# vita-epfl/trajnetplusplusbaselines

Hardware: NVIDIA H100
Metric: pedestrian-steps/sec (higher is better)
Workload: dtype f32

## Files before the change

trajnetplusplusbaselines_b200/csrc/gates_tc.cu:

```cuda
#include <cuda.h>
#include <cuda_bf16.h>
#include <math_constants.h>
#include <cstdio>
#include <cstdlib>
#include <vector>

#include "common.cuh"
#include "wgmma.cuh"

namespace tb2 {

constexpr int kGtBM = 128;
constexpr int kGtBN = 256;
constexpr int kGtBK = 64;
constexpr int kGtStages = 2;
constexpr int kGtThreads = 384;
constexpr int kGtConsumerWarps = 8;
constexpr uint32_t kGtABytes = kGtBM * kGtBK * 2;
constexpr uint32_t kGtBBytes = kGtBN * kGtBK * 2;
constexpr uint32_t kGtStageBytes = 2 * kGtABytes + 2 * kGtBBytes;

__device__ __forceinline__ float g_sigmoid(float x) { return __fdividef(1.f, 1.f + __expf(-x)); }
__device__ __forceinline__ float g_tanh(float x) { return 1.f - __fdividef(2.f, __expf(2.f * x) + 1.f); }

struct GateTcParams {
    const float2* obs1;
    const float2* obs2;
    const float* h_in;
    const float* c_in;
    float* h_out;
    float* c_out;
    __nv_bfloat16* hs_out_hi;
    __nv_bfloat16* hs_out_lo;
    float* normal_out;
    float2* pos_out;
    const float* bg;
    const float* Wn;
    const float* bn;
    int M, P;
    int G;
};

template <int R, bool kGoal>
__global__ void __launch_bounds__(kGtThreads, 1)
lstm_gates_tc_kernel(const __grid_constant__ CUtensorMap map_emb_hi, const __grid_constant__ CUtensorMap map_emb_lo,
                     const __grid_constant__ CUtensorMap map_pool_hi, const __grid_constant__ CUtensorMap map_pool_lo,
                     const __grid_constant__ CUtensorMap map_h_hi, const __grid_constant__ CUtensorMap map_h_lo,
                     const __grid_constant__ CUtensorMap map_w_hi, const __grid_constant__ CUtensorMap map_w_lo,
                     GateTcParams p) {
    extern __shared__ __align__(1024) unsigned char smem_gt[];
    __shared__ __align__(8) uint64_t full_bar[kGtStages];
    __shared__ __align__(8) uint64_t empty_bar[kGtStages];
    __shared__ float wn_s[5][64];
    __shared__ float bg_s[4][64];
    constexpr int H = 64 * R;
    __shared__ float peer_part[R > 1 ? R - 1 : 1][kGtBM][5];

    const int wg = threadIdx.x >> 7, warp = threadIdx.x >> 5, lane = threadIdx.x & 31;
    const int rank = blockIdx.x;
    const int m0 = blockIdx.y * kGtBM;
    const int kb_pool = p.P / kGtBK;
    const int kb_emb = kGoal ? (64 + p.G) / kGtBK : 1;
    const int num_kb = kb_emb + kb_pool + H / kGtBK;
    const uint32_t ring = (smem_u32(smem_gt) + 1023u) & ~1023u;

    for (int i = threadIdx.x; i < 5 * 64; i += kGtThreads) wn_s[i / 64][i % 64] = p.Wn[(i / 64) * H + rank * 64 + (i % 64)];
    for (int i = threadIdx.x; i < 4 * 64; i += kGtThreads) bg_s[i / 64][i % 64] = p.bg[(i / 64) * H + rank * 64 + (i % 64)];

    if (threadIdx.x == 0) {
        for (int s = 0; s < kGtStages; ++s) {
            mbar_init(smem_u32(&full_bar[s]), 1);
            mbar_init(smem_u32(&empty_bar[s]), kGtConsumerWarps);
        }
        asm volatile("fence.mbarrier_init.release.cluster;" ::: "memory");
    }
    __syncthreads();
    grid_dep_wait();
    grid_dep_launch();
    asm volatile("barrier.cluster.arrive.release.aligned;" ::: "memory");
    bool waited_phase1 = false;

    const int rl = wg * 64 + (warp & 3) * 16 + (lane >> 2);
    float part[2][5] = {{0.f, 0.f, 0.f, 0.f, 0.f}, {0.f, 0.f, 0.f, 0.f, 0.f}};

    if (wg == 2) {
        if (threadIdx.x == 256) {
            for (int kb = 0; kb < num_kb; ++kb) {
                const int s = kb % kGtStages;
                const uint32_t phase = (kb / kGtStages) & 1;
                mbar_wait(smem_u32(&empty_bar[s]), phase ^ 1);
                const uint32_t bar = smem_u32(&full_bar[s]);
                const uint32_t base = ring + s * kGtStageBytes;
                mbar_expect_tx(bar, kGtStageBytes);
                const CUtensorMap *ahi, *alo;
                int ka;
                if constexpr (kGoal) {
                    if (kb < kb_emb) { ahi = &map_emb_hi; alo = &map_emb_lo; ka = kb * kGtBK; }
                    else if (kb < kb_emb + kb_pool) { ahi = &map_pool_hi; alo = &map_pool_lo; ka = (kb - kb_emb) * kGtBK; }
                    else { ahi = &map_h_hi; alo = &map_h_lo; ka = (kb - kb_emb - kb_pool) * kGtBK; }
                } else {
                    if (kb == 0) { ahi = &map_emb_hi; alo = &map_emb_lo; ka = 0; }
                    else if (kb <= kb_pool) { ahi = &map_pool_hi; alo = &map_pool_lo; ka = (kb - 1) * kGtBK; }
                    else { ahi = &map_h_hi; alo = &map_h_lo; ka = (kb - 1 - kb_pool) * kGtBK; }
                }
                tma_load_2d(base, ahi, bar, ka, m0);
                tma_load_2d(base + kGtABytes, alo, bar, ka, m0);
                tma_load_2d(base + 2 * kGtABytes, &map_w_hi, bar, kb * kGtBK, rank * kGtBN);
                tma_load_2d(base + 2 * kGtABytes + kGtBBytes, &map_w_lo, bar, kb * kGtBK, rank * kGtBN);
            }
        }
        __syncwarp();
    } else {
        float acc[kGtBN / 2];
#pragma unroll
        for (int i = 0; i < kGtBN / 2; ++i) acc[i] = 0.f;
        const uint32_t a_off = (uint32_t)wg * 64 * 128;
        for (int kb = 0; kb < num_kb; ++kb) {
            const int s = kb % kGtStages;
            const uint32_t phase = (kb / kGtStages) & 1;
            mbar_wait(smem_u32(&full_bar[s]), phase);
            const uint32_t base = ring + s * kGtStageBytes;
            const uint64_t a_hi = wgmma_desc(base + a_off);
            const uint64_t a_lo = wgmma_desc(base + kGtABytes + a_off);
            const uint64_t b_hi = wgmma_desc(base + 2 * kGtABytes);
            const uint64_t b_lo = wgmma_desc(base + 2 * kGtABytes + kGtBBytes);
            wgmma_fence();
#pragma unroll
            for (int k = 0; k < kGtBK / 16; ++k) {
                const uint64_t adv = (uint64_t)((k * 16 * 2) >> 4);
                wgmma_bf16(acc, a_hi + adv, b_hi + adv, (kb | k) != 0);
                wgmma_bf16(acc, a_hi + adv, b_lo + adv, 1u);
                wgmma_bf16(acc, a_lo + adv, b_hi + adv, 1u);
            }
            wgmma_commit();
            wgmma_wait_all();
            if (lane == 0) mbar_arrive(smem_u32(&empty_bar[s]));
        }
#pragma unroll
        for (int hr = 0; hr < 2; ++hr) {
            const int row = m0 + rl + 8 * hr;
            if (row >= p.M) continue;
            const float2 o1 = p.obs1[row], o2 = p.obs2[row];
            const bool masked = isnan(o1.x) || isnan(o2.x);
#pragma unroll
            for (int n8 = 0; n8 < 8; ++n8) {
                const int u = 8 * n8 + 2 * (lane & 3);
                const size_t o = (size_t)row * H + rank * 64 + u;
                float2 c = *reinterpret_cast<const float2*>(p.c_in + o);
                float2 h;
                if (!masked) {
                    float cn[2], hn[2];
                    const float cc[2] = {c.x, c.y};
#pragma unroll
                    for (int j = 0; j < 2; ++j) {
                        const int r = 4 * n8 + 2 * hr + j;
                        const float ig = g_sigmoid(acc[r] + bg_s[0][u + j]);
                        const float fg = g_sigmoid(acc[r + 32] + bg_s[1][u + j]);
                        const float gt = g_tanh(acc[r + 64] + bg_s[2][u + j]);
                        const float og = g_sigmoid(acc[r + 96] + bg_s[3][u + j]);
                        cn[j] = fg * cc[j] + ig * gt;
                        hn[j] = og * g_tanh(cn[j]);
#pragma unroll
                        for (int q = 0; q < 5; ++q) part[hr][q] = fmaf(hn[j], wn_s[q][u + j], part[hr][q]);
                    }
                    c = make_float2(cn[0], cn[1]);
                    h = make_float2(hn[0], hn[1]);
                } else {
                    h = *reinterpret_cast<const float2*>(p.h_in + o);
                }
                *reinterpret_cast<float2*>(p.h_out + o) = h;
                *reinterpret_cast<float2*>(p.c_out + o) = c;
                const __nv_bfloat16 h0 = __float2bfloat16_rn(h.x), h1 = __float2bfloat16_rn(h.y);
                const __nv_bfloat16 l0 = __float2bfloat16_rn(h.x - __bfloat162float(h0));
                const __nv_bfloat16 l1 = __float2bfloat16_rn(h.y - __bfloat162float(h1));
                *reinterpret_cast<uint32_t*>(p.hs_out_hi + o) =
                    (uint32_t)__bfloat16_as_ushort(h0) | ((uint32_t)__bfloat16_as_ushort(h1) << 16);
                *reinterpret_cast<uint32_t*>(p.hs_out_lo + o) =
                    (uint32_t)__bfloat16_as_ushort(l0) | ((uint32_t)__bfloat16_as_ushort(l1) << 16);
            }
        }
#pragma unroll
        for (int hr = 0; hr < 2; ++hr)
#pragma unroll
            for (int q = 0; q < 5; ++q) {
                part[hr][q] += __shfl_xor_sync(0xffffffffu, part[hr][q], 1);
                part[hr][q] += __shfl_xor_sync(0xffffffffu, part[hr][q], 2);
            }
        if (rank > 0) {
            asm volatile("barrier.cluster.wait.acquire.aligned;" ::: "memory");
            waited_phase1 = true;
            if ((lane & 3) == 0) {
#pragma unroll
                for (int hr = 0; hr < 2; ++hr) {
                    const uint32_t local = smem_u32(&peer_part[rank - 1][rl + 8 * hr][0]);
                    uint32_t remote;
                    asm volatile("mapa.shared::cluster.u32 %0, %1, %2;" : "=r"(remote) : "r"(local), "r"(0));
#pragma unroll
                    for (int q = 0; q < 5; ++q)
                        asm volatile("st.shared::cluster.f32 [%0], %1;" ::"r"(remote + 4 * q), "f"(part[hr][q]) : "memory");
                }
            }
            __syncwarp();
        }
    }
    if (!waited_phase1) asm volatile("barrier.cluster.wait.acquire.aligned;" ::: "memory");
    asm volatile("barrier.cluster.arrive.release.aligned;" ::: "memory");
    asm volatile("barrier.cluster.wait.acquire.aligned;" ::: "memory");
    if (wg < 2 && rank == 0 && (lane & 3) == 0) {
#pragma unroll
        for (int hr = 0; hr < 2; ++hr) {
            const int row = m0 + rl + 8 * hr;
            if (row >= p.M) continue;
            float* no = p.normal_out + (size_t)row * 5;
            const float2 o1 = p.obs1[row], o2 = p.obs2[row];
            if (isnan(o1.x) || isnan(o2.x)) {
#pragma unroll
                for (int q = 0; q < 5; ++q) no[q] = CUDART_NAN_F;
                if (p.pos_out) p.pos_out[row] = make_float2(CUDART_NAN_F, CUDART_NAN_F);
            } else {
                float s[5];
#pragma unroll
                for (int q = 0; q < 5; ++q) {
                    s[q] = part[hr][q];
#pragma unroll
                    for (int r = 1; r < R; ++r) s[q] += peer_part[r - 1][rl + 8 * hr][q];
                    s[q] += p.bn[q];
                }
                const float n0 = s[0], n1 = s[1];
                no[0] = n0;
                no[1] = n1;
                no[2] = 0.01f + 0.2f * g_sigmoid(s[2]);
                no[3] = 0.01f + 0.2f * g_sigmoid(s[3]);
                no[4] = 0.7f * g_sigmoid(s[4]);
                if (p.pos_out) p.pos_out[row] = make_float2(o2.x + n0, o2.y + n1);
            }
        }
    }
}

struct GoalEmbed {
    const float2* goals;
    const float* Wg;
    const float* bg;
    int G;
};

template <bool kGoal>
__global__ void embed_split_kernel(const float2* __restrict__ obs1, const float2* __restrict__ obs2,
                                   const float* __restrict__ We, const float* __restrict__ be,
                                   __nv_bfloat16* __restrict__ hi, __nv_bfloat16* __restrict__ lo, int M, int E,
                                   GoalEmbed ge) {
    grid_dep_wait();
    grid_dep_launch();
    const int idx = blockIdx.x * blockDim.x + threadIdx.x;
    const int W = kGoal ? E + ge.G : E;
    if (idx >= M * W) return;
    const int m = idx / W, k = idx - m * W;
    const float2 a = obs1[m], b = obs2[m];
    float v = 0.f;
    if (k < E - 2 && !(isnan(a.x) || isnan(b.x))) {
        const float vx = (b.x - a.x) * 4.0f, vy = (b.y - a.y) * 4.0f;
        v = fmaxf(fmaf(We[2 * k + 1], vy, fmaf(We[2 * k], vx, be[k])), 0.f);
    } else if (kGoal && k >= E && k < W - 2 && !(isnan(a.x) || isnan(b.x))) {
        const int kg = k - E;
        const float2 g = ge.goals[m];
        const float dx = b.x - g.x, dy = b.y - g.y;
        const float n = sqrtf(dx * dx + dy * dy);
        const float gx = n != 0.f ? dx / n : 0.f, gy = n != 0.f ? dy / n : 0.f;
        v = fmaxf(fmaf(ge.Wg[2 * kg + 1], gy * 4.0f, fmaf(ge.Wg[2 * kg], gx * 4.0f, ge.bg[kg])), 0.f);
    }
    const __nv_bfloat16 h = __float2bfloat16_rn(v);
    hi[idx] = h;
    lo[idx] = __float2bfloat16_rn(v - __bfloat162float(h));
}

__global__ void repack_gates_tc_kernel(const float* __restrict__ w_ih, const float* __restrict__ w_hh,
                                       __nv_bfloat16* __restrict__ hi, __nv_bfloat16* __restrict__ lo,
                                       int in_dim, int H) {
    const int K = in_dim + H;
    size_t total = (size_t)4 * H * K;
    for (size_t idx = (size_t)blockIdx.x * blockDim.x + threadIdx.x; idx < total;
         idx += (size_t)gridDim.x * blockDim.x) {
        const int k = (int)(idx % K);
        const int n = (int)(idx / K);
        const int rank = n / 256, gate = (n % 256) / 64, ul = n % 64;
        const int src = gate * H + rank * 64 + ul;
        const float v = k < in_dim ? w_ih[(size_t)src * in_dim + k] : w_hh[(size_t)src * H + (k - in_dim)];
        const __nv_bfloat16 h = __float2bfloat16_rn(v);
        hi[idx] = h;
        lo[idx] = __float2bfloat16_rn(v - __bfloat162float(h));
    }
}

int make_bf16_tile_map(CUtensorMap* map, const void* base, int rows, int cols, int box_rows);

bool gates_tc_supported(const tb2_lstm* m) {
    if (m->H % 64 != 0 || m->E != 64 || (m->E + m->G) % kGtBK != 0) return false;
    if (m->cfg.pool_type != TB2_POOL_NONE && !m->cfg.pool_to_input) return false;
    if (m->P % kGtBK != 0) return false;
    return true;
}

int launch_repack_gates_tc(const float* w_ih, const float* w_hh, void* hi, void* lo, int in_dim, int H,
                           cudaStream_t st) {
    repack_gates_tc_kernel<<<512, 256, 0, st>>>(w_ih, w_hh, (__nv_bfloat16*)hi, (__nv_bfloat16*)lo, in_dim, H);
    TB2_LAUNCH_CHECK();
    return TB2_OK;
}

int launch_embed_split(const tb2_lstm* m, int M, const float* obs1, const float* obs2, const float* goals, void* hi,
                       void* lo, cudaStream_t st) {
    const int total = M * (m->E + m->G);
    const GoalEmbed ge{(const float2*)goals, m->Wgl, m->bgl, m->G};
    {
        KernelTimer kt("embed_split", st);
        launch_pdl(m->G > 0 ? embed_split_kernel<true> : embed_split_kernel<false>, dim3((total + 255) / 256), dim3(256), 0,
                   st, (const float2*)obs1, (const float2*)obs2, (const float*)m->We, (const float*)m->be,
                   (__nv_bfloat16*)hi, (__nv_bfloat16*)lo, M, m->E, ge);
    }
    TB2_LAUNCH_CHECK();
    return TB2_OK;
}

template <int R, bool kGoal>
static int launch_gates_tc_k(const CUtensorMap& me_hi, const CUtensorMap& me_lo, const CUtensorMap& mp_hi,
                             const CUtensorMap& mp_lo, const CUtensorMap& mh_hi, const CUtensorMap& mh_lo,
                             const CUtensorMap& mw_hi, const CUtensorMap& mw_lo, const GateTcParams& p, cudaStream_t st) {
    const size_t smem = (size_t)kGtStages * kGtStageBytes + 1024;
    static DynSmemConfig configured;
    TB2_CHECK_CUDA(configured.ensure(lstm_gates_tc_kernel<R, kGoal>, smem));
    dim3 grid(R, (p.M + kGtBM - 1) / kGtBM);
    {
        KernelTimer kt("lstm_gates_tc", st);
        launch_pdl_cluster(lstm_gates_tc_kernel<R, kGoal>, grid, dim3(kGtThreads), smem, st, (unsigned)R, me_hi, me_lo,
                           mp_hi, mp_lo, mh_hi, mh_lo, mw_hi, mw_lo, p);
    }
    TB2_LAUNCH_CHECK();
    return TB2_OK;
}

template <int R>
static int launch_gates_tc_t(const CUtensorMap& me_hi, const CUtensorMap& me_lo, const CUtensorMap& mp_hi,
                             const CUtensorMap& mp_lo, const CUtensorMap& mh_hi, const CUtensorMap& mh_lo,
                             const CUtensorMap& mw_hi, const CUtensorMap& mw_lo, const GateTcParams& p, cudaStream_t st) {
    return p.G > 0 ? launch_gates_tc_k<R, true>(me_hi, me_lo, mp_hi, mp_lo, mh_hi, mh_lo, mw_hi, mw_lo, p, st)
                   : launch_gates_tc_k<R, false>(me_hi, me_lo, mp_hi, mp_lo, mh_hi, mh_lo, mw_hi, mw_lo, p, st);
}

int launch_gates_tc(const tb2_lstm* m, const tb2_layout* l, int phase, const float* obs1, const float* obs2,
                    const void* emb_hi, const void* emb_lo, const void* pool_hi, const void* pool_lo,
                    const void* hs_in_hi, const void* hs_in_lo, void* hs_out_hi, void* hs_out_lo,
                    const float* h_in, const float* c_in, float* h_out, float* c_out, float* normal_out,
                    float* pos_out, cudaStream_t st) {
    const int M = l->M;
    CUtensorMap me_hi, me_lo, mp_hi, mp_lo, mh_hi, mh_lo, mw_hi, mw_lo;
    int rc;
    if ((rc = make_bf16_tile_map(&me_hi, emb_hi, M, 64 + m->G, kGtBM))) return rc;
    if ((rc = make_bf16_tile_map(&me_lo, emb_lo, M, 64 + m->G, kGtBM))) return rc;
    if (m->P > 0) {
        if ((rc = make_bf16_tile_map(&mp_hi, pool_hi, M, m->P, kGtBM))) return rc;
        if ((rc = make_bf16_tile_map(&mp_lo, pool_lo, M, m->P, kGtBM))) return rc;
    } else {
        mp_hi = me_hi;
        mp_lo = me_lo;
    }
    if ((rc = make_bf16_tile_map(&mh_hi, hs_in_hi, M, m->H, kGtBM))) return rc;
    if ((rc = make_bf16_tile_map(&mh_lo, hs_in_lo, M, m->H, kGtBM))) return rc;
    if ((rc = make_bf16_tile_map(&mw_hi, m->Wg_hi[phase], 4 * m->H, m->K_gate, kGtBN))) return rc;
    if ((rc = make_bf16_tile_map(&mw_lo, m->Wg_lo[phase], 4 * m->H, m->K_gate, kGtBN))) return rc;
    GateTcParams p;
    p.obs1 = (const float2*)obs1;
    p.obs2 = (const float2*)obs2;
    p.h_in = h_in; p.c_in = c_in; p.h_out = h_out; p.c_out = c_out;
    p.hs_out_hi = (__nv_bfloat16*)hs_out_hi; p.hs_out_lo = (__nv_bfloat16*)hs_out_lo;
    p.normal_out = normal_out;
    p.pos_out = (float2*)pos_out;
    p.bg = m->bg[phase];
    p.Wn = m->Wn;
    p.bn = m->bn;
    p.M = M;
    p.P = m->P;
    p.G = m->G;
    switch (m->H) {
        case 64: return launch_gates_tc_t<1>(me_hi, me_lo, mp_hi, mp_lo, mh_hi, mh_lo, mw_hi, mw_lo, p, st);
        case 128: return launch_gates_tc_t<2>(me_hi, me_lo, mp_hi, mp_lo, mh_hi, mh_lo, mw_hi, mw_lo, p, st);
        case 192: return launch_gates_tc_t<3>(me_hi, me_lo, mp_hi, mp_lo, mh_hi, mh_lo, mw_hi, mw_lo, p, st);
        case 256: return launch_gates_tc_t<4>(me_hi, me_lo, mp_hi, mp_lo, mh_hi, mh_lo, mw_hi, mw_lo, p, st);
        default: break;
    }
    set_error(kHiddenDimMessage);
    return TB2_ERR_UNSUPPORTED;
}

}
```

trajnetplusplusbaselines_b200/csrc/gemm_tc.cu:

```cuda
#include <cuda.h>
#include <cuda_bf16.h>
#include <algorithm>

#include "common.cuh"
#include "wgmma.cuh"

namespace tb2 {

constexpr int kTcBM = 128;
constexpr int kTcBK = 64;
constexpr int kTcThreads = 384;
constexpr int kTcConsumerWarps = 8;
constexpr uint32_t kTcABytes = kTcBM * kTcBK * 2;
template <int BN> struct TcCfg {
    static constexpr uint32_t kBBytes = BN * kTcBK * 2;
    static constexpr uint32_t kStageBytes = 2 * kTcABytes + 2 * kBBytes;
    static constexpr int kStages = BN == 128 ? 3 : 4;
};

struct TcParams {
    const float* bias;
    float* Y;
    __nv_bfloat16* Y_hi;
    __nv_bfloat16* Y_lo;
    int M, N, K, relu;
};

__device__ __forceinline__ uint32_t pack_bf16x2(unsigned short a, unsigned short b) { return (uint32_t)a | ((uint32_t)b << 16); }

template <int kTcBN>
__global__ void __launch_bounds__(kTcThreads, 1)
dense_layer_tc_kernel(const __grid_constant__ CUtensorMap map_a_hi, const __grid_constant__ CUtensorMap map_a_lo,
                      const __grid_constant__ CUtensorMap map_b_hi, const __grid_constant__ CUtensorMap map_b_lo,
                      TcParams p) {
    constexpr int kTcStages = TcCfg<kTcBN>::kStages;
    constexpr uint32_t kTcBBytes = TcCfg<kTcBN>::kBBytes;
    constexpr uint32_t kTcStageBytes = TcCfg<kTcBN>::kStageBytes;
    extern __shared__ __align__(1024) unsigned char smem_tc[];
    __shared__ __align__(8) uint64_t full_bar[kTcStages];
    __shared__ __align__(8) uint64_t empty_bar[kTcStages];

    const int wg = threadIdx.x >> 7, warp = threadIdx.x >> 5, lane = threadIdx.x & 31;
    const int m0 = blockIdx.y * kTcBM, n0 = blockIdx.x * kTcBN;
    const int num_kb = p.K / kTcBK;
    const uint32_t ring = (smem_u32(smem_tc) + 1023u) & ~1023u;

    if (threadIdx.x == 0) {
        asm volatile("prefetch.tensormap [%0];" ::"l"(&map_a_hi) : "memory");
        asm volatile("prefetch.tensormap [%0];" ::"l"(&map_a_lo) : "memory");
        asm volatile("prefetch.tensormap [%0];" ::"l"(&map_b_hi) : "memory");
        asm volatile("prefetch.tensormap [%0];" ::"l"(&map_b_lo) : "memory");
        for (int s = 0; s < kTcStages; ++s) {
            mbar_init(smem_u32(&full_bar[s]), 1);
            mbar_init(smem_u32(&empty_bar[s]), kTcConsumerWarps);
        }
        asm volatile("fence.mbarrier_init.release.cluster;" ::: "memory");
    }
    __syncthreads();
    grid_dep_wait();
    grid_dep_launch();

    if (wg == 2) {
        if (threadIdx.x == 256) {
            for (int kb = 0; kb < num_kb; ++kb) {
                const int s = kb % kTcStages;
                const uint32_t phase = (kb / kTcStages) & 1;
                mbar_wait(smem_u32(&empty_bar[s]), phase ^ 1);
                const uint32_t bar = smem_u32(&full_bar[s]);
                const uint32_t base = ring + s * kTcStageBytes;
                mbar_expect_tx(bar, kTcStageBytes);
                tma_load_2d(base, &map_a_hi, bar, kb * kTcBK, m0);
                tma_load_2d(base + kTcABytes, &map_a_lo, bar, kb * kTcBK, m0);
                tma_load_2d(base + 2 * kTcABytes, &map_b_hi, bar, kb * kTcBK, n0);
                tma_load_2d(base + 2 * kTcABytes + kTcBBytes, &map_b_lo, bar, kb * kTcBK, n0);
            }
        }
        return;
    }
    float acc[kTcBN / 2];
#pragma unroll
    for (int i = 0; i < kTcBN / 2; ++i) acc[i] = 0.f;
    const uint32_t a_off = (uint32_t)wg * 64 * 128;
    for (int kb = 0; kb < num_kb; ++kb) {
        const int s = kb % kTcStages;
        const uint32_t phase = (kb / kTcStages) & 1;
        mbar_wait(smem_u32(&full_bar[s]), phase);
        const uint32_t base = ring + s * kTcStageBytes;
        const uint64_t a_hi = wgmma_desc(base + a_off);
        const uint64_t a_lo = wgmma_desc(base + kTcABytes + a_off);
        const uint64_t b_hi = wgmma_desc(base + 2 * kTcABytes);
        const uint64_t b_lo = wgmma_desc(base + 2 * kTcABytes + kTcBBytes);
        wgmma_fence();
#pragma unroll
        for (int k = 0; k < kTcBK / 16; ++k) {
            const uint64_t adv = (uint64_t)((k * 16 * 2) >> 4);
            wgmma_bf16(acc, a_hi + adv, b_hi + adv, (kb | k) != 0);
            wgmma_bf16(acc, a_hi + adv, b_lo + adv, 1u);
            wgmma_bf16(acc, a_lo + adv, b_hi + adv, 1u);
        }
        wgmma_commit();
        wgmma_wait_all();
        if (lane == 0) mbar_arrive(smem_u32(&empty_bar[s]));
    }
    const int row0 = m0 + wg * 64 + (warp & 3) * 16 + (lane >> 2);
    const int col0 = n0 + 2 * (lane & 3);
#pragma unroll
    for (int i = 0; i < kTcBN / 2; i += 2) {
        const int gr = row0 + 8 * ((i >> 1) & 1);
        const int gc = col0 + 8 * (i >> 2);
        float v0 = acc[i] + p.bias[gc], v1 = acc[i + 1] + p.bias[gc + 1];
        if (p.relu) { v0 = fmaxf(v0, 0.f); v1 = fmaxf(v1, 0.f); }
        if (gr >= p.M) continue;
        const size_t yoff = (size_t)gr * p.N + gc;
        if (p.Y) *reinterpret_cast<float2*>(p.Y + yoff) = make_float2(v0, v1);
        if (p.Y_hi) {
            const __nv_bfloat16 h0 = __float2bfloat16_rn(v0), h1 = __float2bfloat16_rn(v1);
            *reinterpret_cast<uint32_t*>(p.Y_hi + yoff) = pack_bf16x2(__bfloat16_as_ushort(h0), __bfloat16_as_ushort(h1));
            *reinterpret_cast<uint32_t*>(p.Y_lo + yoff) =
                pack_bf16x2(__bfloat16_as_ushort(__float2bfloat16_rn(v0 - __bfloat162float(h0))),
                            __bfloat16_as_ushort(__float2bfloat16_rn(v1 - __bfloat162float(h1))));
        }
    }
}

typedef CUresult (*EncodeTiledFn)(CUtensorMap*, CUtensorMapDataType, cuuint32_t, void*, const cuuint64_t*,
                                  const cuuint64_t*, const cuuint32_t*, const cuuint32_t*, CUtensorMapInterleave,
                                  CUtensorMapSwizzle, CUtensorMapL2promotion, CUtensorMapFloatOOBfill);

static EncodeTiledFn encode_fn() {
    static EncodeTiledFn fn = nullptr;
    if (!fn) {
        void* p = nullptr;
        cudaDriverEntryPointQueryResult q;
        if (cudaGetDriverEntryPoint("cuTensorMapEncodeTiled", &p, cudaEnableDefault, &q) == cudaSuccess &&
            q == cudaDriverEntryPointSuccess)
            fn = (EncodeTiledFn)p;
    }
    return fn;
}

int make_bf16_tile_map(CUtensorMap* map, const void* base, int rows, int cols, int box_rows) {
    struct Entry { const void* base; int rows, cols, box_rows; bool valid; CUtensorMap map; };
    static thread_local Entry cache[256] = {};
    const uintptr_t key = reinterpret_cast<uintptr_t>(base);
    Entry& e = cache[((key >> 8) ^ (key >> 17) ^ (uintptr_t)(rows * 131 + cols * 7 + box_rows)) & 255];
    if (e.valid && e.base == base && e.rows == rows && e.cols == cols && e.box_rows == box_rows) {
        *map = e.map;
        return TB2_OK;
    }
    EncodeTiledFn fn = encode_fn();
    if (!fn) { set_error("cuTensorMapEncodeTiled unavailable"); return TB2_ERR_CUDA; }
    cuuint64_t dims[2] = {(cuuint64_t)cols, (cuuint64_t)rows};
    cuuint64_t strides[1] = {(cuuint64_t)cols * 2};
    cuuint32_t box[2] = {(cuuint32_t)kTcBK, (cuuint32_t)box_rows};
    cuuint32_t estr[2] = {1, 1};
    CUresult r = fn(map, CU_TENSOR_MAP_DATA_TYPE_BFLOAT16, 2, const_cast<void*>(base), dims, strides, box, estr,
                    CU_TENSOR_MAP_INTERLEAVE_NONE, CU_TENSOR_MAP_SWIZZLE_128B, CU_TENSOR_MAP_L2_PROMOTION_L2_256B,
                    CU_TENSOR_MAP_FLOAT_OOB_FILL_NONE);
    if (r != CUDA_SUCCESS) { set_error("cuTensorMapEncodeTiled failed (" + std::to_string((int)r) + ")"); return TB2_ERR_CUDA; }
    e.base = base; e.rows = rows; e.cols = cols; e.box_rows = box_rows; e.map = *map; e.valid = true;
    return TB2_OK;
}

bool dense_tc_supported(int K, int N) { return K >= kTcBK && K % kTcBK == 0 && N % 64 == 0; }

template <int BN>
static int launch_dense_tc_t(const CUtensorMap& ma_hi, const CUtensorMap& ma_lo, const CUtensorMap& mb_hi,
                             const CUtensorMap& mb_lo, const TcParams& p, cudaStream_t st) {
    const size_t smem = (size_t)TcCfg<BN>::kStages * TcCfg<BN>::kStageBytes + 1024;
    static DynSmemConfig configured;
    TB2_CHECK_CUDA(configured.ensure(dense_layer_tc_kernel<BN>, smem));
    dim3 grid(p.N / BN, (p.M + kTcBM - 1) / kTcBM);
    {
        KernelTimer kt("dense_layer_tc", st);
        launch_pdl(dense_layer_tc_kernel<BN>, grid, dim3(kTcThreads), smem, st, ma_hi, ma_lo, mb_hi, mb_lo, p);
    }
    TB2_LAUNCH_CHECK();
    return TB2_OK;
}

int launch_dense_tc(const void* a_hi, const void* a_lo, const void* w_hi, const void* w_lo, const float* bias,
                    float* Y, void* Y_hi, void* Y_lo, int M, int K, int N, int relu, cudaStream_t st) {
    TB2_REQUIRE(dense_tc_supported(K, N), "tensor-core dense layer needs K % 64 == 0 and N % 64 == 0");
    CUtensorMap ma_hi, ma_lo, mb_hi, mb_lo;
    int rc;
    if ((rc = make_bf16_tile_map(&ma_hi, a_hi, M, K, kTcBM))) return rc;
    if ((rc = make_bf16_tile_map(&ma_lo, a_lo, M, K, kTcBM))) return rc;
    const int bn = (N % 128 == 0) ? 128 : 64;
    if ((rc = make_bf16_tile_map(&mb_hi, w_hi, N, K, bn))) return rc;
    if ((rc = make_bf16_tile_map(&mb_lo, w_lo, N, K, bn))) return rc;
    TcParams p;
    p.bias = bias;
    p.Y = Y;
    p.Y_hi = (__nv_bfloat16*)Y_hi;
    p.Y_lo = (__nv_bfloat16*)Y_lo;
    p.M = M;
    p.N = N;
    p.K = K;
    p.relu = relu;
    return bn == 128 ? launch_dense_tc_t<128>(ma_hi, ma_lo, mb_hi, mb_lo, p, st)
                     : launch_dense_tc_t<64>(ma_hi, ma_lo, mb_hi, mb_lo, p, st);
}

__global__ void split_bf16_kernel(const float* __restrict__ src, __nv_bfloat16* __restrict__ hi,
                                  __nv_bfloat16* __restrict__ lo, size_t n) {
    for (size_t i = (size_t)blockIdx.x * blockDim.x + threadIdx.x; i < n; i += (size_t)gridDim.x * blockDim.x) {
        const float v = src[i];
        const __nv_bfloat16 h = __float2bfloat16_rn(v);
        hi[i] = h;
        lo[i] = __float2bfloat16_rn(v - __bfloat162float(h));
    }
}

int launch_split_bf16(const float* src, void* hi, void* lo, size_t n, cudaStream_t st) {
    if (n == 0) return TB2_OK;
    const unsigned blocks = (unsigned)std::min<size_t>((n + 255) / 256, 1184);
    split_bf16_kernel<<<blocks, 256, 0, st>>>(src, (__nv_bfloat16*)hi, (__nv_bfloat16*)lo, n);
    TB2_LAUNCH_CHECK();
    return TB2_OK;
}

}
```

trajnetplusplusbaselines_b200/csrc/wgmma.cuh:

```cuda
#pragma once
#include <cuda.h>
#include <stdint.h>

namespace tb2 {

__device__ __forceinline__ uint32_t smem_u32(const void* p) { return (uint32_t)__cvta_generic_to_shared(p); }

__device__ __forceinline__ void mbar_init(uint32_t bar, uint32_t count) {
    asm volatile("mbarrier.init.shared::cta.b64 [%0], %1;" ::"r"(bar), "r"(count));
}
__device__ __forceinline__ void mbar_expect_tx(uint32_t bar, uint32_t bytes) {
    asm volatile("mbarrier.arrive.expect_tx.shared::cta.b64 _, [%0], %1;" ::"r"(bar), "r"(bytes) : "memory");
}
__device__ __forceinline__ void mbar_arrive(uint32_t bar) {
    asm volatile("mbarrier.arrive.shared::cta.b64 _, [%0];" ::"r"(bar) : "memory");
}
__device__ __forceinline__ void mbar_wait(uint32_t bar, uint32_t parity) {
    asm volatile(
        "{\n"
        ".reg .pred p;\n"
        "WAIT_LOOP:\n"
        "mbarrier.try_wait.parity.shared::cta.b64 p, [%0], %1;\n"
        "@p bra WAIT_DONE;\n"
        "bra WAIT_LOOP;\n"
        "WAIT_DONE:\n"
        "}\n" ::"r"(bar), "r"(parity) : "memory");
}
__device__ __forceinline__ void tma_load_2d(uint32_t dst, const CUtensorMap* map, uint32_t bar, int c0, int c1) {
    asm volatile(
        "cp.async.bulk.tensor.2d.shared::cluster.global.mbarrier::complete_tx::bytes [%0], [%1, {%3, %4}], [%2];"
        ::"r"(dst), "l"(map), "r"(bar), "r"(c0), "r"(c1) : "memory");
}

__device__ __forceinline__ uint64_t wgmma_desc(uint32_t smem_addr) {
    uint64_t d = 0;
    d |= (uint64_t)((smem_addr & 0x3FFFF) >> 4);
    d |= (uint64_t)1 << 16;
    d |= (uint64_t)(1024 >> 4) << 32;
    d |= (uint64_t)1 << 62;
    return d;
}
__device__ __forceinline__ void wgmma_fence() { asm volatile("wgmma.fence.sync.aligned;" ::: "memory"); }
__device__ __forceinline__ void wgmma_commit() { asm volatile("wgmma.commit_group.sync.aligned;" ::: "memory"); }
__device__ __forceinline__ void wgmma_wait_all() { asm volatile("wgmma.wait_group.sync.aligned 0;" ::: "memory"); }

__device__ __forceinline__ void wgmma_bf16(float (&d)[32], uint64_t a, uint64_t b, uint32_t accumulate) {
    asm volatile(
        "{\n"
        ".reg .pred p;\n"
        "setp.ne.b32 p, %34, 0;\n"
        "wgmma.mma_async.sync.aligned.m64n64k16.f32.bf16.bf16 "
        "{%0, %1, %2, %3, %4, %5, %6, %7, %8, %9, %10, %11, %12, %13, %14, %15, %16, %17, %18, %19, %20, %21, %22, %23, %24, %25, %26, %27, %28, %29, %30, %31}, "
        "%32, %33, p, 1, 1, 0, 0;\n"
        "}\n"
        : "+f"(d[0]), "+f"(d[1]), "+f"(d[2]), "+f"(d[3]), "+f"(d[4]), "+f"(d[5]), "+f"(d[6]), "+f"(d[7]),
          "+f"(d[8]), "+f"(d[9]), "+f"(d[10]), "+f"(d[11]), "+f"(d[12]), "+f"(d[13]), "+f"(d[14]), "+f"(d[15]),
          "+f"(d[16]), "+f"(d[17]), "+f"(d[18]), "+f"(d[19]), "+f"(d[20]), "+f"(d[21]), "+f"(d[22]), "+f"(d[23]),
          "+f"(d[24]), "+f"(d[25]), "+f"(d[26]), "+f"(d[27]), "+f"(d[28]), "+f"(d[29]), "+f"(d[30]), "+f"(d[31])
        : "l"(a), "l"(b), "r"(accumulate));
}
__device__ __forceinline__ void wgmma_bf16(float (&d)[64], uint64_t a, uint64_t b, uint32_t accumulate) {
    asm volatile(
        "{\n"
        ".reg .pred p;\n"
        "setp.ne.b32 p, %66, 0;\n"
        "wgmma.mma_async.sync.aligned.m64n128k16.f32.bf16.bf16 "
        "{%0, %1, %2, %3, %4, %5, %6, %7, %8, %9, %10, %11, %12, %13, %14, %15, %16, %17, %18, %19, %20, %21, %22, %23, %24, %25, %26, %27, %28, %29, %30, %31, %32, %33, %34, %35, %36, %37, %38, %39, %40, %41, %42, %43, %44, %45, %46, %47, %48, %49, %50, %51, %52, %53, %54, %55, %56, %57, %58, %59, %60, %61, %62, %63}, "
        "%64, %65, p, 1, 1, 0, 0;\n"
        "}\n"
        : "+f"(d[0]), "+f"(d[1]), "+f"(d[2]), "+f"(d[3]), "+f"(d[4]), "+f"(d[5]), "+f"(d[6]), "+f"(d[7]),
          "+f"(d[8]), "+f"(d[9]), "+f"(d[10]), "+f"(d[11]), "+f"(d[12]), "+f"(d[13]), "+f"(d[14]), "+f"(d[15]),
          "+f"(d[16]), "+f"(d[17]), "+f"(d[18]), "+f"(d[19]), "+f"(d[20]), "+f"(d[21]), "+f"(d[22]), "+f"(d[23]),
          "+f"(d[24]), "+f"(d[25]), "+f"(d[26]), "+f"(d[27]), "+f"(d[28]), "+f"(d[29]), "+f"(d[30]), "+f"(d[31]),
          "+f"(d[32]), "+f"(d[33]), "+f"(d[34]), "+f"(d[35]), "+f"(d[36]), "+f"(d[37]), "+f"(d[38]), "+f"(d[39]),
          "+f"(d[40]), "+f"(d[41]), "+f"(d[42]), "+f"(d[43]), "+f"(d[44]), "+f"(d[45]), "+f"(d[46]), "+f"(d[47]),
          "+f"(d[48]), "+f"(d[49]), "+f"(d[50]), "+f"(d[51]), "+f"(d[52]), "+f"(d[53]), "+f"(d[54]), "+f"(d[55]),
          "+f"(d[56]), "+f"(d[57]), "+f"(d[58]), "+f"(d[59]), "+f"(d[60]), "+f"(d[61]), "+f"(d[62]), "+f"(d[63])
        : "l"(a), "l"(b), "r"(accumulate));
}
__device__ __forceinline__ void wgmma_bf16(float (&d)[128], uint64_t a, uint64_t b, uint32_t accumulate) {
    asm volatile(
        "{\n"
        ".reg .pred p;\n"
        "setp.ne.b32 p, %130, 0;\n"
        "wgmma.mma_async.sync.aligned.m64n256k16.f32.bf16.bf16 "
        "{%0, %1, %2, %3, %4, %5, %6, %7, %8, %9, %10, %11, %12, %13, %14, %15, %16, %17, %18, %19, %20, %21, %22, %23, %24, %25, %26, %27, %28, %29, %30, %31, %32, %33, %34, %35, %36, %37, %38, %39, %40, %41, %42, %43, %44, %45, %46, %47, %48, %49, %50, %51, %52, %53, %54, %55, %56, %57, %58, %59, %60, %61, %62, %63, %64, %65, %66, %67, %68, %69, %70, %71, %72, %73, %74, %75, %76, %77, %78, %79, %80, %81, %82, %83, %84, %85, %86, %87, %88, %89, %90, %91, %92, %93, %94, %95, %96, %97, %98, %99, %100, %101, %102, %103, %104, %105, %106, %107, %108, %109, %110, %111, %112, %113, %114, %115, %116, %117, %118, %119, %120, %121, %122, %123, %124, %125, %126, %127}, "
        "%128, %129, p, 1, 1, 0, 0;\n"
        "}\n"
        : "+f"(d[0]), "+f"(d[1]), "+f"(d[2]), "+f"(d[3]), "+f"(d[4]), "+f"(d[5]), "+f"(d[6]), "+f"(d[7]),
          "+f"(d[8]), "+f"(d[9]), "+f"(d[10]), "+f"(d[11]), "+f"(d[12]), "+f"(d[13]), "+f"(d[14]), "+f"(d[15]),
          "+f"(d[16]), "+f"(d[17]), "+f"(d[18]), "+f"(d[19]), "+f"(d[20]), "+f"(d[21]), "+f"(d[22]), "+f"(d[23]),
          "+f"(d[24]), "+f"(d[25]), "+f"(d[26]), "+f"(d[27]), "+f"(d[28]), "+f"(d[29]), "+f"(d[30]), "+f"(d[31]),
          "+f"(d[32]), "+f"(d[33]), "+f"(d[34]), "+f"(d[35]), "+f"(d[36]), "+f"(d[37]), "+f"(d[38]), "+f"(d[39]),
          "+f"(d[40]), "+f"(d[41]), "+f"(d[42]), "+f"(d[43]), "+f"(d[44]), "+f"(d[45]), "+f"(d[46]), "+f"(d[47]),
          "+f"(d[48]), "+f"(d[49]), "+f"(d[50]), "+f"(d[51]), "+f"(d[52]), "+f"(d[53]), "+f"(d[54]), "+f"(d[55]),
          "+f"(d[56]), "+f"(d[57]), "+f"(d[58]), "+f"(d[59]), "+f"(d[60]), "+f"(d[61]), "+f"(d[62]), "+f"(d[63]),
          "+f"(d[64]), "+f"(d[65]), "+f"(d[66]), "+f"(d[67]), "+f"(d[68]), "+f"(d[69]), "+f"(d[70]), "+f"(d[71]),
          "+f"(d[72]), "+f"(d[73]), "+f"(d[74]), "+f"(d[75]), "+f"(d[76]), "+f"(d[77]), "+f"(d[78]), "+f"(d[79]),
          "+f"(d[80]), "+f"(d[81]), "+f"(d[82]), "+f"(d[83]), "+f"(d[84]), "+f"(d[85]), "+f"(d[86]), "+f"(d[87]),
          "+f"(d[88]), "+f"(d[89]), "+f"(d[90]), "+f"(d[91]), "+f"(d[92]), "+f"(d[93]), "+f"(d[94]), "+f"(d[95]),
          "+f"(d[96]), "+f"(d[97]), "+f"(d[98]), "+f"(d[99]), "+f"(d[100]), "+f"(d[101]), "+f"(d[102]), "+f"(d[103]),
          "+f"(d[104]), "+f"(d[105]), "+f"(d[106]), "+f"(d[107]), "+f"(d[108]), "+f"(d[109]), "+f"(d[110]), "+f"(d[111]),
          "+f"(d[112]), "+f"(d[113]), "+f"(d[114]), "+f"(d[115]), "+f"(d[116]), "+f"(d[117]), "+f"(d[118]), "+f"(d[119]),
          "+f"(d[120]), "+f"(d[121]), "+f"(d[122]), "+f"(d[123]), "+f"(d[124]), "+f"(d[125]), "+f"(d[126]), "+f"(d[127])
        : "l"(a), "l"(b), "r"(accumulate));
}

}
```

Measured before the change: 31.13 million.

## Deepen gate GEMM pipeline with smaller K tiles, prefetch epilogue inputs, stage outputs

The LSTM gate kernel switches to 32-wide K blocks with three pipeline stages and 64-byte swizzle, which needs a templated wgmma descriptor and a box-column parameter on the tensor map builder. Its c_in and observation rows are prefetched into shared memory with cp.async during the GEMM, so the epilogue reads shared memory instead of global. The dense GEMM now caches bias in shared memory and stages outputs in the ring buffer so the f32 and bf16 hi/lo results go out as coalesced vector stores. Compile-time ablation switches (TB2_GEMM_ABLATE) are added and default to off. Smaller K blocks mean more barrier round-trips per tile, and the extra shared buffers raise shared-memory use.

```diff
diff --git a/trajnetplusplusbaselines_b200/csrc/gates_tc.cu b/trajnetplusplusbaselines_b200/csrc/gates_tc.cu
--- a/trajnetplusplusbaselines_b200/csrc/gates_tc.cu
+++ b/trajnetplusplusbaselines_b200/csrc/gates_tc.cu
@@ -12,8 +12,8 @@
 
 constexpr int kGtBM = 128;
 constexpr int kGtBN = 256;
-constexpr int kGtBK = 64;
-constexpr int kGtStages = 2;
+constexpr int kGtBK = 32;
+constexpr int kGtStages = 3;
 constexpr int kGtThreads = 384;
 constexpr int kGtConsumerWarps = 8;
 constexpr uint32_t kGtABytes = kGtBM * kGtBK * 2;
@@ -55,12 +55,14 @@
     __shared__ float bg_s[4][64];
     constexpr int H = 64 * R;
     __shared__ float peer_part[R > 1 ? R - 1 : 1][kGtBM][5];
+    __shared__ float2 c_s[16][256];
+    __shared__ float2 obs_s[kGtBM][2];
 
     const int wg = threadIdx.x >> 7, warp = threadIdx.x >> 5, lane = threadIdx.x & 31;
     const int rank = blockIdx.x;
     const int m0 = blockIdx.y * kGtBM;
     const int kb_pool = p.P / kGtBK;
-    const int kb_emb = kGoal ? (64 + p.G) / kGtBK : 1;
+    const int kb_emb = (64 + (kGoal ? p.G : 0)) / kGtBK;
     const int num_kb = kb_emb + kb_pool + H / kGtBK;
     const uint32_t ring = (smem_u32(smem_gt) + 1023u) & ~1023u;
 
@@ -81,11 +83,30 @@
     bool waited_phase1 = false;
 
     const int rl = wg * 64 + (warp & 3) * 16 + (lane >> 2);
+    if (wg < 2) {
+#pragma unroll
+        for (int hr = 0; hr < 2; ++hr) {
+            const int row = m0 + rl + 8 * hr;
+            if (row >= p.M) continue;
+            if ((lane & 3) == 0) {
+                asm volatile("cp.async.ca.shared.global [%0], [%1], 8;"
+                             ::"r"(smem_u32(&obs_s[rl + 8 * hr][0])), "l"(p.obs1 + row) : "memory");
+                asm volatile("cp.async.ca.shared.global [%0], [%1], 8;"
+                             ::"r"(smem_u32(&obs_s[rl + 8 * hr][1])), "l"(p.obs2 + row) : "memory");
+            }
+#pragma unroll
+            for (int n8 = 0; n8 < 8; ++n8)
+                asm volatile("cp.async.ca.shared.global [%0], [%1], 8;"
+                             ::"r"(smem_u32(&c_s[8 * hr + n8][threadIdx.x])),
+                               "l"(p.c_in + (size_t)row * H + rank * 64 + 8 * n8 + 2 * (lane & 3)) : "memory");
+        }
+        asm volatile("cp.async.commit_group;" ::: "memory");
+    }
     float part[2][5] = {{0.f, 0.f, 0.f, 0.f, 0.f}, {0.f, 0.f, 0.f, 0.f, 0.f}};
 
     if (wg == 2) {
         if (threadIdx.x == 256) {
-            for (int kb = 0; kb < num_kb; ++kb) {
+            for (int kb = 0; kb < (TB2_GEMM_ABLATE == 2 ? 1 : num_kb); ++kb) {
                 const int s = kb % kGtStages;
                 const uint32_t phase = (kb / kGtStages) & 1;
                 mbar_wait(smem_u32(&empty_bar[s]), phase ^ 1);
@@ -94,15 +115,9 @@
                 mbar_expect_tx(bar, kGtStageBytes);
                 const CUtensorMap *ahi, *alo;
                 int ka;
-                if constexpr (kGoal) {
-                    if (kb < kb_emb) { ahi = &map_emb_hi; alo = &map_emb_lo; ka = kb * kGtBK; }
-                    else if (kb < kb_emb + kb_pool) { ahi = &map_pool_hi; alo = &map_pool_lo; ka = (kb - kb_emb) * kGtBK; }
-                    else { ahi = &map_h_hi; alo = &map_h_lo; ka = (kb - kb_emb - kb_pool) * kGtBK; }
-                } else {
-                    if (kb == 0) { ahi = &map_emb_hi; alo = &map_emb_lo; ka = 0; }
-                    else if (kb <= kb_pool) { ahi = &map_pool_hi; alo = &map_pool_lo; ka = (kb - 1) * kGtBK; }
-                    else { ahi = &map_h_hi; alo = &map_h_lo; ka = (kb - 1 - kb_pool) * kGtBK; }
-                }
+                if (kb < kb_emb) { ahi = &map_emb_hi; alo = &map_emb_lo; ka = kb * kGtBK; }
+                else if (kb < kb_emb + kb_pool) { ahi = &map_pool_hi; alo = &map_pool_lo; ka = (kb - kb_emb) * kGtBK; }
+                else { ahi = &map_h_hi; alo = &map_h_lo; ka = (kb - kb_emb - kb_pool) * kGtBK; }
                 tma_load_2d(base, ahi, bar, ka, m0);
                 tma_load_2d(base + kGtABytes, alo, bar, ka, m0);
                 tma_load_2d(base + 2 * kGtABytes, &map_w_hi, bar, kb * kGtBK, rank * kGtBN);
@@ -114,39 +129,47 @@
         float acc[kGtBN / 2];
 #pragma unroll
         for (int i = 0; i < kGtBN / 2; ++i) acc[i] = 0.f;
-        const uint32_t a_off = (uint32_t)wg * 64 * 128;
+        const uint32_t a_off = (uint32_t)wg * 64 * 2 * kGtBK;
         for (int kb = 0; kb < num_kb; ++kb) {
-            const int s = kb % kGtStages;
-            const uint32_t phase = (kb / kGtStages) & 1;
+            const int s = TB2_GEMM_ABLATE == 2 ? 0 : kb % kGtStages;
+            const uint32_t phase = TB2_GEMM_ABLATE == 2 ? 0 : (kb / kGtStages) & 1;
             mbar_wait(smem_u32(&full_bar[s]), phase);
             const uint32_t base = ring + s * kGtStageBytes;
-            const uint64_t a_hi = wgmma_desc(base + a_off);
-            const uint64_t a_lo = wgmma_desc(base + kGtABytes + a_off);
-            const uint64_t b_hi = wgmma_desc(base + 2 * kGtABytes);
-            const uint64_t b_lo = wgmma_desc(base + 2 * kGtABytes + kGtBBytes);
+            const uint64_t a_hi = wgmma_desc<2 * kGtBK>(base + a_off);
+            const uint64_t a_lo = wgmma_desc<2 * kGtBK>(base + kGtABytes + a_off);
+            const uint64_t b_hi = wgmma_desc<2 * kGtBK>(base + 2 * kGtABytes);
+            const uint64_t b_lo = wgmma_desc<2 * kGtBK>(base + 2 * kGtABytes + kGtBBytes);
             wgmma_fence();
 #pragma unroll
-            for (int k = 0; k < kGtBK / 16; ++k) {
+            for (int k = 0; k < (TB2_GEMM_ABLATE == 1 ? 0 : kGtBK / 16); ++k) {
                 const uint64_t adv = (uint64_t)((k * 16 * 2) >> 4);
                 wgmma_bf16(acc, a_hi + adv, b_hi + adv, (kb | k) != 0);
                 wgmma_bf16(acc, a_hi + adv, b_lo + adv, 1u);
                 wgmma_bf16(acc, a_lo + adv, b_hi + adv, 1u);
             }
             wgmma_commit();
-            wgmma_wait_all();
+#if TB2_GEMM_ABLATE == 4
+            wgmma_wait<1>();
+            if (kb > 0 && lane == 0) mbar_arrive(smem_u32(&empty_bar[(kb - 1) % kGtStages]));
+#else
+            wgmma_wait<0>();
             if (lane == 0) mbar_arrive(smem_u32(&empty_bar[s]));
-        }
+#endif
+        }
+        wgmma_wait<0>();
+        asm volatile("cp.async.wait_group 0;" ::: "memory");
+        asm volatile("bar.sync 1, 256;" ::: "memory");
 #pragma unroll
         for (int hr = 0; hr < 2; ++hr) {
             const int row = m0 + rl + 8 * hr;
-            if (row >= p.M) continue;
-            const float2 o1 = p.obs1[row], o2 = p.obs2[row];
+            if (row >= p.M || (TB2_GEMM_ABLATE == 3 && p.M > 0)) continue;
+            const float2 o1 = obs_s[rl + 8 * hr][0], o2 = obs_s[rl + 8 * hr][1];
             const bool masked = isnan(o1.x) || isnan(o2.x);
 #pragma unroll
             for (int n8 = 0; n8 < 8; ++n8) {
                 const int u = 8 * n8 + 2 * (lane & 3);
                 const size_t o = (size_t)row * H + rank * 64 + u;
-                float2 c = *reinterpret_cast<const float2*>(p.c_in + o);
+                float2 c = c_s[8 * hr + n8][threadIdx.x];
                 float2 h;
                 if (!masked) {
                     float cn[2], hn[2];
@@ -210,9 +233,9 @@
 #pragma unroll
         for (int hr = 0; hr < 2; ++hr) {
             const int row = m0 + rl + 8 * hr;
-            if (row >= p.M) continue;
+            if (row >= p.M || (TB2_GEMM_ABLATE == 3 && p.M > 0)) continue;
             float* no = p.normal_out + (size_t)row * 5;
-            const float2 o1 = p.obs1[row], o2 = p.obs2[row];
+            const float2 o1 = obs_s[rl + 8 * hr][0], o2 = obs_s[rl + 8 * hr][1];
             if (isnan(o1.x) || isnan(o2.x)) {
 #pragma unroll
                 for (int q = 0; q < 5; ++q) no[q] = CUDART_NAN_F;
@@ -292,12 +315,12 @@
     }
 }
 
-int make_bf16_tile_map(CUtensorMap* map, const void* base, int rows, int cols, int box_rows);
+int make_bf16_tile_map(CUtensorMap* map, const void* base, int rows, int cols, int box_rows, int box_cols);
 
 bool gates_tc_supported(const tb2_lstm* m) {
-    if (m->H % 64 != 0 || m->E != 64 || (m->E + m->G) % kGtBK != 0) return false;
+    if (m->H % 64 != 0 || m->E != 64 || (m->E + m->G) % 64 != 0) return false;
     if (m->cfg.pool_type != TB2_POOL_NONE && !m->cfg.pool_to_input) return false;
-    if (m->P % kGtBK != 0) return false;
+    if (m->P % 64 != 0) return false;
     return true;
 }
 
@@ -355,19 +378,19 @@
     const int M = l->M;
     CUtensorMap me_hi, me_lo, mp_hi, mp_lo, mh_hi, mh_lo, mw_hi, mw_lo;
     int rc;
-    if ((rc = make_bf16_tile_map(&me_hi, emb_hi, M, 64 + m->G, kGtBM))) return rc;
-    if ((rc = make_bf16_tile_map(&me_lo, emb_lo, M, 64 + m->G, kGtBM))) return rc;
+    if ((rc = make_bf16_tile_map(&me_hi, emb_hi, M, 64 + m->G, kGtBM, kGtBK))) return rc;
+    if ((rc = make_bf16_tile_map(&me_lo, emb_lo, M, 64 + m->G, kGtBM, kGtBK))) return rc;
     if (m->P > 0) {
-        if ((rc = make_bf16_tile_map(&mp_hi, pool_hi, M, m->P, kGtBM))) return rc;
-        if ((rc = make_bf16_tile_map(&mp_lo, pool_lo, M, m->P, kGtBM))) return rc;
+        if ((rc = make_bf16_tile_map(&mp_hi, pool_hi, M, m->P, kGtBM, kGtBK))) return rc;
+        if ((rc = make_bf16_tile_map(&mp_lo, pool_lo, M, m->P, kGtBM, kGtBK))) return rc;
     } else {
         mp_hi = me_hi;
         mp_lo = me_lo;
     }
-    if ((rc = make_bf16_tile_map(&mh_hi, hs_in_hi, M, m->H, kGtBM))) return rc;
-    if ((rc = make_bf16_tile_map(&mh_lo, hs_in_lo, M, m->H, kGtBM))) return rc;
-    if ((rc = make_bf16_tile_map(&mw_hi, m->Wg_hi[phase], 4 * m->H, m->K_gate, kGtBN))) return rc;
-    if ((rc = make_bf16_tile_map(&mw_lo, m->Wg_lo[phase], 4 * m->H, m->K_gate, kGtBN))) return rc;
+    if ((rc = make_bf16_tile_map(&mh_hi, hs_in_hi, M, m->H, kGtBM, kGtBK))) return rc;
+    if ((rc = make_bf16_tile_map(&mh_lo, hs_in_lo, M, m->H, kGtBM, kGtBK))) return rc;
+    if ((rc = make_bf16_tile_map(&mw_hi, m->Wg_hi[phase], 4 * m->H, m->K_gate, kGtBN, kGtBK))) return rc;
+    if ((rc = make_bf16_tile_map(&mw_lo, m->Wg_lo[phase], 4 * m->H, m->K_gate, kGtBN, kGtBK))) return rc;
     GateTcParams p;
     p.obs1 = (const float2*)obs1;
     p.obs2 = (const float2*)obs2;
diff --git a/trajnetplusplusbaselines_b200/csrc/gemm_tc.cu b/trajnetplusplusbaselines_b200/csrc/gemm_tc.cu
--- a/trajnetplusplusbaselines_b200/csrc/gemm_tc.cu
+++ b/trajnetplusplusbaselines_b200/csrc/gemm_tc.cu
@@ -39,6 +39,7 @@
     extern __shared__ __align__(1024) unsigned char smem_tc[];
     __shared__ __align__(8) uint64_t full_bar[kTcStages];
     __shared__ __align__(8) uint64_t empty_bar[kTcStages];
+    __shared__ float bias_s[kTcBN];
 
     const int wg = threadIdx.x >> 7, warp = threadIdx.x >> 5, lane = threadIdx.x & 31;
     const int m0 = blockIdx.y * kTcBM, n0 = blockIdx.x * kTcBN;
@@ -62,7 +63,7 @@
 
     if (wg == 2) {
         if (threadIdx.x == 256) {
-            for (int kb = 0; kb < num_kb; ++kb) {
+            for (int kb = 0; kb < (TB2_GEMM_ABLATE == 2 ? 1 : num_kb); ++kb) {
                 const int s = kb % kTcStages;
                 const uint32_t phase = (kb / kTcStages) & 1;
                 mbar_wait(smem_u32(&empty_bar[s]), phase ^ 1);
@@ -77,13 +78,14 @@
         }
         return;
     }
+    if (threadIdx.x < kTcBN) bias_s[threadIdx.x] = p.bias[n0 + threadIdx.x];
     float acc[kTcBN / 2];
 #pragma unroll
     for (int i = 0; i < kTcBN / 2; ++i) acc[i] = 0.f;
     const uint32_t a_off = (uint32_t)wg * 64 * 128;
     for (int kb = 0; kb < num_kb; ++kb) {
-        const int s = kb % kTcStages;
-        const uint32_t phase = (kb / kTcStages) & 1;
+        const int s = TB2_GEMM_ABLATE == 2 ? 0 : kb % kTcStages;
+        const uint32_t phase = TB2_GEMM_ABLATE == 2 ? 0 : (kb / kTcStages) & 1;
         mbar_wait(smem_u32(&full_bar[s]), phase);
         const uint32_t base = ring + s * kTcStageBytes;
         const uint64_t a_hi = wgmma_desc(base + a_off);
@@ -92,33 +94,63 @@
         const uint64_t b_lo = wgmma_desc(base + 2 * kTcABytes + kTcBBytes);
         wgmma_fence();
 #pragma unroll
-        for (int k = 0; k < kTcBK / 16; ++k) {
+        for (int k = 0; k < (TB2_GEMM_ABLATE == 1 ? 0 : kTcBK / 16); ++k) {
             const uint64_t adv = (uint64_t)((k * 16 * 2) >> 4);
             wgmma_bf16(acc, a_hi + adv, b_hi + adv, (kb | k) != 0);
             wgmma_bf16(acc, a_hi + adv, b_lo + adv, 1u);
             wgmma_bf16(acc, a_lo + adv, b_hi + adv, 1u);
         }
         wgmma_commit();
-        wgmma_wait_all();
+#if TB2_GEMM_ABLATE == 4
+        wgmma_wait<1>();
+        if (kb > 0 && lane == 0) mbar_arrive(smem_u32(&empty_bar[(kb - 1) % kTcStages]));
+#else
+        wgmma_wait<0>();
         if (lane == 0) mbar_arrive(smem_u32(&empty_bar[s]));
-    }
-    const int row0 = m0 + wg * 64 + (warp & 3) * 16 + (lane >> 2);
-    const int col0 = n0 + 2 * (lane & 3);
+#endif
+    }
+    wgmma_wait<0>();
+    asm volatile("bar.sync 1, 256;" ::: "memory");
+    constexpr int kYStride = kTcBN + 8;
+    constexpr int kHStride = kTcBN + 16;
+    static_assert(kTcBM * (kYStride * 4 + 2 * kHStride * 2) <= kTcStages * kTcStageBytes, "output tiles fit the ring");
+    float* y_s = reinterpret_cast<float*>(smem_tc + (ring - smem_u32(smem_tc)));
+    uint32_t* hi_s = reinterpret_cast<uint32_t*>(y_s + kTcBM * kYStride);
+    uint32_t* lo_s = hi_s + kTcBM * kHStride / 2;
+    const int r0 = wg * 64 + (warp & 3) * 16 + (lane >> 2);
+    const int c0 = 2 * (lane & 3);
 #pragma unroll
     for (int i = 0; i < kTcBN / 2; i += 2) {
-        const int gr = row0 + 8 * ((i >> 1) & 1);
-        const int gc = col0 + 8 * (i >> 2);
-        float v0 = acc[i] + p.bias[gc], v1 = acc[i + 1] + p.bias[gc + 1];
+        const int r = r0 + 8 * ((i >> 1) & 1);
+        const int c = c0 + 8 * (i >> 2);
+        float v0 = acc[i] + bias_s[c], v1 = acc[i + 1] + bias_s[c + 1];
         if (p.relu) { v0 = fmaxf(v0, 0.f); v1 = fmaxf(v1, 0.f); }
-        if (gr >= p.M) continue;
-        const size_t yoff = (size_t)gr * p.N + gc;
-        if (p.Y) *reinterpret_cast<float2*>(p.Y + yoff) = make_float2(v0, v1);
-        if (p.Y_hi) {
-            const __nv_bfloat16 h0 = __float2bfloat16_rn(v0), h1 = __float2bfloat16_rn(v1);
-            *reinterpret_cast<uint32_t*>(p.Y_hi + yoff) = pack_bf16x2(__bfloat16_as_ushort(h0), __bfloat16_as_ushort(h1));
-            *reinterpret_cast<uint32_t*>(p.Y_lo + yoff) =
-                pack_bf16x2(__bfloat16_as_ushort(__float2bfloat16_rn(v0 - __bfloat162float(h0))),
-                            __bfloat16_as_ushort(__float2bfloat16_rn(v1 - __bfloat162float(h1))));
+        *reinterpret_cast<float2*>(y_s + r * kYStride + c) = make_float2(v0, v1);
+        const __nv_bfloat16 h0 = __float2bfloat16_rn(v0), h1 = __float2bfloat16_rn(v1);
+        hi_s[(r * kHStride + c) / 2] = pack_bf16x2(__bfloat16_as_ushort(h0), __bfloat16_as_ushort(h1));
+        lo_s[(r * kHStride + c) / 2] = pack_bf16x2(__bfloat16_as_ushort(__float2bfloat16_rn(v0 - __bfloat162float(h0))),
+                                                   __bfloat16_as_ushort(__float2bfloat16_rn(v1 - __bfloat162float(h1))));
+    }
+    asm volatile("bar.sync 1, 256;" ::: "memory");
+    if (TB2_GEMM_ABLATE == 3 && p.M > 0) return;
+    if (p.Y) {
+        constexpr int kChunks = kTcBN / 4;
+        for (int q = threadIdx.x; q < kTcBM * kChunks; q += 256) {
+            const int r = q / kChunks, c = 4 * (q % kChunks);
+            if (m0 + r < p.M)
+                *reinterpret_cast<float4*>(p.Y + (size_t)(m0 + r) * p.N + n0 + c) =
+                    *reinterpret_cast<const float4*>(y_s + r * kYStride + c);
+        }
+    }
+    if (p.Y_hi) {
+        constexpr int kChunks = kTcBN / 8;
+        for (int q = threadIdx.x; q < kTcBM * kChunks; q += 256) {
+            const int r = q / kChunks, c = 8 * (q % kChunks);
+            if (m0 + r < p.M) {
+                const size_t o = (size_t)(m0 + r) * p.N + n0 + c;
+                *reinterpret_cast<uint4*>(p.Y_hi + o) = *reinterpret_cast<const uint4*>(hi_s + (r * kHStride + c) / 2);
+                *reinterpret_cast<uint4*>(p.Y_lo + o) = *reinterpret_cast<const uint4*>(lo_s + (r * kHStride + c) / 2);
+            }
         }
     }
 }
@@ -139,12 +171,13 @@
     return fn;
 }
 
-int make_bf16_tile_map(CUtensorMap* map, const void* base, int rows, int cols, int box_rows) {
-    struct Entry { const void* base; int rows, cols, box_rows; bool valid; CUtensorMap map; };
+int make_bf16_tile_map(CUtensorMap* map, const void* base, int rows, int cols, int box_rows, int box_cols) {
+    struct Entry { const void* base; int rows, cols, box_rows, box_cols; bool valid; CUtensorMap map; };
     static thread_local Entry cache[256] = {};
     const uintptr_t key = reinterpret_cast<uintptr_t>(base);
-    Entry& e = cache[((key >> 8) ^ (key >> 17) ^ (uintptr_t)(rows * 131 + cols * 7 + box_rows)) & 255];
-    if (e.valid && e.base == base && e.rows == rows && e.cols == cols && e.box_rows == box_rows) {
+    Entry& e = cache[((key >> 8) ^ (key >> 17) ^ (uintptr_t)(rows * 131 + cols * 7 + box_rows + box_cols)) & 255];
+    if (e.valid && e.base == base && e.rows == rows && e.cols == cols && e.box_rows == box_rows &&
+        e.box_cols == box_cols) {
         *map = e.map;
         return TB2_OK;
     }
@@ -152,13 +185,15 @@
     if (!fn) { set_error("cuTensorMapEncodeTiled unavailable"); return TB2_ERR_CUDA; }
     cuuint64_t dims[2] = {(cuuint64_t)cols, (cuuint64_t)rows};
     cuuint64_t strides[1] = {(cuuint64_t)cols * 2};
-    cuuint32_t box[2] = {(cuuint32_t)kTcBK, (cuuint32_t)box_rows};
+    cuuint32_t box[2] = {(cuuint32_t)box_cols, (cuuint32_t)box_rows};
     cuuint32_t estr[2] = {1, 1};
     CUresult r = fn(map, CU_TENSOR_MAP_DATA_TYPE_BFLOAT16, 2, const_cast<void*>(base), dims, strides, box, estr,
-                    CU_TENSOR_MAP_INTERLEAVE_NONE, CU_TENSOR_MAP_SWIZZLE_128B, CU_TENSOR_MAP_L2_PROMOTION_L2_256B,
+                    CU_TENSOR_MAP_INTERLEAVE_NONE, box_cols == 64 ? CU_TENSOR_MAP_SWIZZLE_128B : CU_TENSOR_MAP_SWIZZLE_64B,
+                    CU_TENSOR_MAP_L2_PROMOTION_L2_256B,
                     CU_TENSOR_MAP_FLOAT_OOB_FILL_NONE);
     if (r != CUDA_SUCCESS) { set_error("cuTensorMapEncodeTiled failed (" + std::to_string((int)r) + ")"); return TB2_ERR_CUDA; }
-    e.base = base; e.rows = rows; e.cols = cols; e.box_rows = box_rows; e.map = *map; e.valid = true;
+    e.base = base; e.rows = rows; e.cols = cols; e.box_rows = box_rows; e.box_cols = box_cols; e.map = *map;
+    e.valid = true;
     return TB2_OK;
 }
 
@@ -184,11 +219,11 @@
     TB2_REQUIRE(dense_tc_supported(K, N), "tensor-core dense layer needs K % 64 == 0 and N % 64 == 0");
     CUtensorMap ma_hi, ma_lo, mb_hi, mb_lo;
     int rc;
-    if ((rc = make_bf16_tile_map(&ma_hi, a_hi, M, K, kTcBM))) return rc;
-    if ((rc = make_bf16_tile_map(&ma_lo, a_lo, M, K, kTcBM))) return rc;
+    if ((rc = make_bf16_tile_map(&ma_hi, a_hi, M, K, kTcBM, kTcBK))) return rc;
+    if ((rc = make_bf16_tile_map(&ma_lo, a_lo, M, K, kTcBM, kTcBK))) return rc;
     const int bn = (N % 128 == 0) ? 128 : 64;
-    if ((rc = make_bf16_tile_map(&mb_hi, w_hi, N, K, bn))) return rc;
-    if ((rc = make_bf16_tile_map(&mb_lo, w_lo, N, K, bn))) return rc;
+    if ((rc = make_bf16_tile_map(&mb_hi, w_hi, N, K, bn, kTcBK))) return rc;
+    if ((rc = make_bf16_tile_map(&mb_lo, w_lo, N, K, bn, kTcBK))) return rc;
     TcParams p;
     p.bias = bias;
     p.Y = Y;
diff --git a/trajnetplusplusbaselines_b200/csrc/wgmma.cuh b/trajnetplusplusbaselines_b200/csrc/wgmma.cuh
--- a/trajnetplusplusbaselines_b200/csrc/wgmma.cuh
+++ b/trajnetplusplusbaselines_b200/csrc/wgmma.cuh
@@ -1,6 +1,10 @@
 #pragma once
 #include <cuda.h>
 #include <stdint.h>
+
+#ifndef TB2_GEMM_ABLATE
+#define TB2_GEMM_ABLATE 0
+#endif
 
 namespace tb2 {
 
@@ -32,17 +36,20 @@
         ::"r"(dst), "l"(map), "r"(bar), "r"(c0), "r"(c1) : "memory");
 }
 
+template <int kRowBytes = 128>
 __device__ __forceinline__ uint64_t wgmma_desc(uint32_t smem_addr) {
+    static_assert(kRowBytes == 128 || kRowBytes == 64, "128- or 64-byte swizzled rows");
     uint64_t d = 0;
     d |= (uint64_t)((smem_addr & 0x3FFFF) >> 4);
     d |= (uint64_t)1 << 16;
-    d |= (uint64_t)(1024 >> 4) << 32;
-    d |= (uint64_t)1 << 62;
+    d |= (uint64_t)(8 * kRowBytes >> 4) << 32;
+    d |= (uint64_t)(kRowBytes == 128 ? 1 : 2) << 62;
     return d;
 }
 __device__ __forceinline__ void wgmma_fence() { asm volatile("wgmma.fence.sync.aligned;" ::: "memory"); }
 __device__ __forceinline__ void wgmma_commit() { asm volatile("wgmma.commit_group.sync.aligned;" ::: "memory"); }
-__device__ __forceinline__ void wgmma_wait_all() { asm volatile("wgmma.wait_group.sync.aligned 0;" ::: "memory"); }
+template <int N>
+__device__ __forceinline__ void wgmma_wait() { asm volatile("wgmma.wait_group.sync.aligned %0;" ::"n"(N) : "memory"); }
 
 __device__ __forceinline__ void wgmma_bf16(float (&d)[32], uint64_t a, uint64_t b, uint32_t accumulate) {
     asm volatile(
```

Result: faster. 32.54 million, median of 6 (+4.5%).
